# cloudtik/cloudtik

Hardware: AMD Instinct MI355X
Metric: bert_large_pretrain_tokens_per_sec (higher is better)
Workload: dtype bf16

## Files before the change

### cloudtik_amd/ops/csrc/bindings_lt.cpp

```cpp
#include <torch/extension.h>
#include <ATen/hip/HIPContext.h>
#include <ATen/hip/HIPContextLight.h>
#include <hipblaslt/hipblaslt.h>
#include <hipblaslt/hipblaslt-ext.hpp>
#include <map>
#include <vector>
#include <mutex>
#include <tuple>

namespace {

#define LT_CHECK(x)                                                                     \
  do {                                                                                  \
    hipblasStatus_t st_ = (x);                                                          \
    TORCH_CHECK(st_ == HIPBLAS_STATUS_SUCCESS, "hipBLASLt: ", #x, " failed: ", (int)st_); \
  } while (0)

using Key = std::tuple<long, long, long, long, long, long, long, long, long, int, int, int, int, int>;

struct Plan {
  hipblasLtMatmulDesc_t desc = nullptr;
  hipblasLtMatrixLayout_t a = nullptr, b = nullptr, c = nullptr, d = nullptr;
  hipblasLtMatmulAlgo_t algo;
  size_t ws = 0;
// ... 223 lines not shown
      tuned_ms = p.ok ? best : -1.0;
      it = g_bplans.emplace(key, p).first;
    }
    plan = &it->second;
  }
  if (!plan->ok) return -1.0;
  LT_CHECK(hipblasLtMatmul(handle, plan->desc, &al, B.data_ptr(), plan->a, A.data_ptr(), plan->b, &be, D.data_ptr(),
                           plan->d, D.data_ptr(), plan->d, &plan->algo, ws, plan->ws, stream));
  return tuned_ms;
}

extern "C" int ct_gemm_nt(const void*, long, const void*, long, void*, long, int, int, int, int, int, const void*,
                          void*, long, float*, int, hipStream_t, int);

static bool gemm_nt_impl(at::Tensor A, at::Tensor B, at::Tensor D, int64_t epi, bool accumulate,
                         c10::optional<at::Tensor> bias, c10::optional<at::Tensor> aux, c10::optional<at::Tensor> dbias,
                         bool b_kn) {
  TORCH_CHECK(A.is_cuda() && B.is_cuda() && D.is_cuda(), "gemm_nt: GPU tensors");
  TORCH_CHECK(A.scalar_type() == at::kBFloat16 && B.scalar_type() == at::kBFloat16 &&
              D.scalar_type() == at::kBFloat16, "gemm_nt: bf16 operands");
  TORCH_CHECK(rowmajor_ok(A) && rowmajor_ok(B) && rowmajor_ok(D), "gemm_nt: 2-D row-major operands");
  const long M = A.size(0), K = A.size(1), N = b_kn ? B.size(1) : B.size(0);
  TORCH_CHECK((b_kn ? B.size(0) : B.size(1)) == K && D.size(0) == M && D.size(1) == N, "gemm_nt: shape mismatch");
  const bool hb = bias.has_value() && bias->defined(), ha = aux.has_value() && aux->defined(),
             hd = dbias.has_value() && dbias->defined();
  if (hb) TORCH_CHECK(bias->scalar_type() == at::kBFloat16 && bias->is_contiguous() && bias->numel() == N,
                      "gemm_nt: bias");
  if (ha) TORCH_CHECK(aux->scalar_type() == at::kBFloat16 && rowmajor_ok(*aux) && aux->size(0) == M &&
                      aux->size(1) == N, "gemm_nt: aux");
  const long drows = hd && N > 0 ? dbias->numel() / N : 1;
  if (hd) TORCH_CHECK(dbias->scalar_type() == at::kFloat && dbias->is_contiguous() && dbias->numel() == drows * N &&
                      drows >= 1 && (drows & (drows - 1)) == 0, "gemm_nt: dbias must be [N] or [2^k, N] fp32");
  TORCH_CHECK((epi != 1 && epi != 6) || (hb && ha), "gemm_nt: epilogues 1 / 6 need bias and aux");
  TORCH_CHECK((epi != 2 && epi != 7) || ha, "gemm_nt: epilogues 2 / 7 need aux");
  int rc = ct_gemm_nt(A.data_ptr(), A.stride(0), B.data_ptr(), B.stride(0), D.data_ptr(), D.stride(0), (int)M,
                      (int)N, (int)K, (int)epi, accumulate ? 1 : 0, hb ? bias->data_ptr() : nullptr,
                      ha ? aux->data_ptr() : nullptr, ha ? aux->stride(0) : 0,
                      hd ? dbias->data_ptr<float>() : nullptr, b_kn ? 1 : 0, at::hip::getCurrentHIPStream().stream(),
                      (int)drows);
  return rc == 0;
}

bool gemm_nt(at::Tensor A, at::Tensor B, at::Tensor D, int64_t epi, bool accumulate, c10::optional<at::Tensor> bias,
             c10::optional<at::Tensor> aux, c10::optional<at::Tensor> dbias) {
  return gemm_nt_impl(A, B, D, epi, accumulate, bias, aux, dbias, false);
}

bool gemm_nn(at::Tensor A, at::Tensor B, at::Tensor D, int64_t epi, bool accumulate, c10::optional<at::Tensor> bias,
             c10::optional<at::Tensor> aux, c10::optional<at::Tensor> dbias) {
  return gemm_nt_impl(A, B, D, epi, accumulate, bias, aux, dbias, true);
}

extern "C" int ct_gemm_nt_stream(const void*, long, const void*, long, void*, long, int, int, int, int, const void*,
                                 int, int, int, hipStream_t);

bool gemm_nt_stream(at::Tensor A, at::Tensor B, at::Tensor D, c10::optional<at::Tensor> bias, bool b_kn,
                    int64_t wgs, bool accumulate) {
  TORCH_CHECK(A.is_cuda() && B.is_cuda() && D.is_cuda(), "gemm_nt_stream: GPU tensors");
  TORCH_CHECK(A.scalar_type() == at::kBFloat16 && B.scalar_type() == at::kBFloat16 &&
              D.scalar_type() == at::kBFloat16, "gemm_nt_stream: bf16 operands");
  TORCH_CHECK(rowmajor_ok(A) && rowmajor_ok(B) && rowmajor_ok(D), "gemm_nt_stream: 2-D row-major operands");
  const long M = A.size(0), K = A.size(1), N = b_kn ? B.size(1) : B.size(0);
  TORCH_CHECK((b_kn ? B.size(0) : B.size(1)) == K && D.size(0) == M && D.size(1) == N,
              "gemm_nt_stream: shape mismatch");
  const bool hb = bias.has_value() && bias->defined();
  if (hb) TORCH_CHECK(bias->scalar_type() == at::kBFloat16 && bias->is_contiguous() && bias->numel() == N,
                      "gemm_nt_stream: bias");
  int rc = ct_gemm_nt_stream(A.data_ptr(), A.stride(0), B.data_ptr(), B.stride(0), D.data_ptr(), D.stride(0),
                             (int)M, (int)N, (int)K, hb ? 5 : 0, hb ? bias->data_ptr() : nullptr, b_kn ? 1 : 0,
                             (int)wgs, accumulate ? 1 : 0, at::hip::getCurrentHIPStream().stream());
  return rc == 0;
}

extern "C" int ct_gemm_pp(const void*, long, const void*, long, void*, long, int, int, int, int, const void*, void*,
                          long, int, int, hipStream_t);

bool gemm_pp(at::Tensor A, at::Tensor B, at::Tensor D, int64_t epi, c10::optional<at::Tensor> bias,
             c10::optional<at::Tensor> aux, int64_t wgs, int64_t eslots) {
  TORCH_CHECK(A.is_cuda() && B.is_cuda() && D.is_cuda(), "gemm_pp: GPU tensors");
  TORCH_CHECK(A.scalar_type() == at::kBFloat16 && B.scalar_type() == at::kBFloat16 &&
              D.scalar_type() == at::kBFloat16, "gemm_pp: bf16 operands");
  TORCH_CHECK(rowmajor_ok(A) && rowmajor_ok(B) && rowmajor_ok(D), "gemm_pp: 2-D row-major operands");
  const long M = A.size(0), K = A.size(1), N = B.size(0);
  TORCH_CHECK(B.size(1) == K && D.size(0) == M && D.size(1) == N, "gemm_pp: shape mismatch");
  const bool hb = bias.has_value() && bias->defined();
  const bool ha = aux.has_value() && aux->defined();
  if (hb) TORCH_CHECK(bias->scalar_type() == at::kBFloat16 && bias->is_contiguous() && bias->numel() == N,
                      "gemm_pp: bias");
  if (ha) TORCH_CHECK(aux->scalar_type() == at::kBFloat16 && rowmajor_ok(*aux) && aux->size(0) == M &&
                      aux->size(1) == N, "gemm_pp: aux");
  int rc = ct_gemm_pp(A.data_ptr(), A.stride(0), B.data_ptr(), B.stride(0), D.data_ptr(), D.stride(0), (int)M, (int)N,
                      (int)K, (int)epi, hb ? bias->data_ptr() : nullptr, ha ? aux->data_ptr() : nullptr,
                      ha ? aux->stride(0) : 0, (int)wgs, (int)eslots, at::hip::getCurrentHIPStream().stream());
  return rc == 0;
}

extern "C" int ct_gemm_w4(const void*, long, const void*, long, void*, long, int, int, int, int, int, const void*, void*,
                          long, hipStream_t);

bool gemm_w4(at::Tensor A, at::Tensor B, at::Tensor D, int64_t epi, c10::optional<at::Tensor> bias,
             c10::optional<at::Tensor> aux) {
  TORCH_CHECK(A.is_cuda() && B.is_cuda() && D.is_cuda(), "gemm_w4: GPU tensors");
  TORCH_CHECK(A.scalar_type() == at::kBFloat16 && B.scalar_type() == at::kBFloat16 &&
              D.scalar_type() == at::kBFloat16, "gemm_w4: bf16 operands");
  TORCH_CHECK(rowmajor_ok(A) && rowmajor_ok(B) && rowmajor_ok(D), "gemm_w4: 2-D row-major operands");
  const long M = A.size(0), K = A.size(1), N = B.size(0);
  TORCH_CHECK(B.size(1) == K && D.size(0) == M && D.size(1) == N, "gemm_w4: shape mismatch");
  const bool hb = bias.has_value() && bias->defined();
  const bool ha = aux.has_value() && aux->defined();
  if (hb) TORCH_CHECK(bias->scalar_type() == at::kBFloat16 && bias->is_contiguous() && bias->numel() == N,
                      "gemm_w4: bias");
  if (ha) TORCH_CHECK(aux->scalar_type() == at::kBFloat16 && rowmajor_ok(*aux) && aux->size(0) == M &&
                      aux->size(1) == N, "gemm_w4: aux");
  int rc = ct_gemm_w4(A.data_ptr(), A.stride(0), B.data_ptr(), B.stride(0), D.data_ptr(), D.stride(0), (int)M, (int)N,
                      (int)K, (int)epi, 0, hb ? bias->data_ptr() : nullptr, ha ? aux->data_ptr() : nullptr,
                      ha ? aux->stride(0) : 0, at::hip::getCurrentHIPStream().stream());
  return rc == 0;
}

extern "C" int ct_gemm_tn2(const void*, long, const void*, long, void*, long, int, int, long, int, int, float*,
                           hipStream_t);

static void check_tn_problem(const char* who, const at::Tensor& A, const at::Tensor& B, const at::Tensor& out,
// ... 23 lines not shown
                     (int)splits, accumulate ? 1 : 0, biasg, at::hip::getCurrentHIPStream().stream()) == 0;
}

bool gemm_tn2(at::Tensor A, at::Tensor B, at::Tensor out, int64_t splits, bool accumulate) {
  return gemm_tn2_impl(A, B, out, splits, accumulate, nullptr);
}

bool gemm_tn2_bias(at::Tensor A, at::Tensor B, at::Tensor out, int64_t splits, bool accumulate, at::Tensor biasg) {
  TORCH_CHECK(biasg.is_cuda() && biasg.scalar_type() == at::kFloat && biasg.is_contiguous() &&
              biasg.numel() == splits * A.size(1), "gemm_tn2_bias: fp32 [splits, M] bias partials");
  return gemm_tn2_impl(A, B, out, splits, accumulate, biasg.data_ptr<float>());
}

extern "C" int ct_gemm_tn_group(int, const void* const*, const long*, const void* const*, const long*, float* const*,
                                float* const*, const int*, const int*, long, int, hipStream_t);

bool gemm_tn_group(std::vector<at::Tensor> A, std::vector<at::Tensor> B, std::vector<at::Tensor> P,
                   std::vector<c10::optional<at::Tensor>> biasg, int64_t splits) {
  const size_t n = A.size();
  TORCH_CHECK(n >= 1 && B.size() == n && P.size() == n && biasg.size() == n, "gemm_tn_group: list lengths");
  std::vector<const void*> a(n), b(n);
  std::vector<float*> p(n), bg(n);
  std::vector<long> lda(n), ldb(n);
  std::vector<int> Ms(n), Ns(n);
  const long K = A[0].dim() == 2 ? A[0].size(0) : -1;
  for (size_t i = 0; i < n; ++i) {
    check_tn_problem("gemm_tn_group", A[i], B[i], P[i], K, splits, true);
    const long M = A[i].size(1), N = B[i].size(1);
    const bool hb = biasg[i].has_value() && biasg[i]->defined();
    if (hb)
      TORCH_CHECK(biasg[i]->is_cuda() && biasg[i]->scalar_type() == at::kFloat && biasg[i]->is_contiguous() &&
                  biasg[i]->numel() == splits * M, "gemm_tn_group: fp32 [splits, M] bias partials");
    a[i] = A[i].data_ptr();
    b[i] = B[i].data_ptr();
    p[i] = P[i].data_ptr<float>();
    bg[i] = hb ? biasg[i]->data_ptr<float>() : nullptr;
    lda[i] = A[i].stride(0);
    ldb[i] = B[i].stride(0);
    Ms[i] = (int)M;
    Ns[i] = (int)N;
  }
  return ct_gemm_tn_group((int)n, a.data(), lda.data(), b.data(), ldb.data(), p.data(), bg.data(), Ms.data(),
                          Ns.data(), K, (int)std::min<int64_t>(splits, 1 << 30),
                          at::hip::getCurrentHIPStream().stream()) == 0;
}

void register_lt(pybind11::module& m) {
  m.def("gemm_tn_group", &gemm_tn_group, "several gemm_tn2 problems sharing K and the slice count, one launch");
  m.def("gemm_tn2", &gemm_tn2, "weight-gradient GEMM A^T @ B (token-major operands) on the MFMA kernel");
  m.def("gemm_tn2_bias", &gemm_tn2_bias, "gemm_tn2 + per-split column sums of A (bias gradient)");
  m.def("gemm_nt", &gemm_nt, "hand-written MFMA GEMM A @ B^T with fused epilogues");
  m.def("gemm_nt_stream", &gemm_nt_stream, "streamed persistent MFMA GEMM A @ B^T / A @ B (+ bias)",
        pybind11::arg("A"), pybind11::arg("B"), pybind11::arg("D"), pybind11::arg("bias") = pybind11::none(), pybind11::arg("b_kn") = false,
        pybind11::arg("wgs") = 0, pybind11::arg("accumulate") = false);
  m.def("gemm_pp", &gemm_pp, "paired-tile persistent MFMA GEMM A @ B^T (epilogue of one tile beside another's K loop)",
        pybind11::arg("A"), pybind11::arg("B"), pybind11::arg("D"), pybind11::arg("epi") = 0,
        pybind11::arg("bias") = pybind11::none(), pybind11::arg("aux") = pybind11::none(), pybind11::arg("wgs") = 0,
        pybind11::arg("eslots") = 4);
  m.def("gemm_w4", &gemm_w4, "four-wave MFMA GEMM A @ B^T (128 x 128 per wave, AGPR-resident accumulators)",
        pybind11::arg("A"), pybind11::arg("B"), pybind11::arg("D"), pybind11::arg("epi") = 0,
        pybind11::arg("bias") = pybind11::none(), pybind11::arg("aux") = pybind11::none());
  m.def("gemm_nn", &gemm_nn, "hand-written MFMA GEMM A @ B (B stored [K, N]) with fused epilogues");
  m.def("lt_matmul", &lt_matmul, "hipBLASLt matmul with epilogue (row-major semantics)");
  m.def("lt_bmm_tuned", &lt_bmm_tuned, "strided-batched hipBLASLt GEMM, algorithm picked by timing all solutions");
}
```

### cloudtik_amd/ops/csrc/gemm_nt.hip

```cpp
#include "common.h"
#include <algorithm>
#include <cstdlib>

namespace ct {

typedef __attribute__((ext_vector_type(8))) short nt_s16x8;
typedef __attribute__((address_space(3))) nt_s16x8 nt_lds_s16x8;
typedef __attribute__((address_space(3))) void nt_lds_void;

constexpr int NT_BM = 256, NT_BN = 256, NT_BK = 64, NT_THREADS = 512;
constexpr int NT_ROWB = NT_BK * 2;
constexpr int NT_HALF = 128 * NT_ROWB;
constexpr int NT_BUF = 4 * NT_HALF;

enum { NT_EPI_PLAIN = 0, NT_EPI_BIAS_GELU_AUX = 1, NT_EPI_DGELU_BGRAD = 2, NT_EPI_F32_SLAB = 3, NT_EPI_NONE = 4,
       NT_EPI_BIAS = 5, NT_EPI_BIAS_GELU_DAUX = 6, NT_EPI_MUL_AUX_BGRAD = 7 };

struct NtArgs {
  const bf16_t* A;
  const bf16_t* B;
  bf16_t* D;
  const bf16_t* bias;
  bf16_t* aux;
  float* dbias;
// ... 124 lines not shown
    const long krow = c.kbase + k0 + piece * 4;
    const bf16_t* base;
    unsigned off;
    if (slot == 0 || slot == 3) {
      if constexpr (!Ly::AT) {
        base = c.A + (c.m0 + ((piece >> 3) << 7) + (slot == 3 ? 64 : 0) + (piece & 7) * 8) * c.lda + k0;
        off = i ? c.offa1 : c.offa0;
      } else {
        base = c.A + krow * c.lda + c.m0 + (slot == 3 ? 64 : 0);
        off = c.offa0;
      }
    } else {
      if constexpr (!Ly::BT) {
        base = c.B + (c.n0 + ((piece >> 2) << 6) + (slot == 2 ? 32 : 0) + (piece & 3) * 8) * c.ldb + k0;
        off = i ? c.offb1 : c.offb0;
      } else {
        base = c.B + krow * c.ldb + c.n0 + (slot == 2 ? 32 : 0);
        off = c.offb0;
      }
    }
    nt_glds16s(base, off, dst + piece * 1024);
  }
}

template <int N>
__device__ __forceinline__ void nt_vm() {
  asm volatile("s_waitcnt vmcnt(%0)" ::"n"(N) : "memory");
}

template <int I0, int J0>
__device__ __forceinline__ void nt_quad(f32x4 (&acc)[8][4], const nt_s16x8 (&fa)[4][2], const nt_s16x8 (&fb)[2][2]) {
#pragma unroll
  for (int ks = 0; ks < 2; ++ks)
#pragma unroll
    for (int i = 0; i < 4; ++i)
#pragma unroll
      for (int j = 0; j < 2; ++j)
        acc[I0 + i][J0 + j] = __builtin_amdgcn_mfma_f32_16x16x32_bf16((bf16x8_t)fb[j][ks], (bf16x8_t)fa[i][ks],
                                                                       acc[I0 + i][J0 + j], 0, 0, 0);
}

template <int LAY>
__device__ __forceinline__ void nt_stage_v(const NtCtx& c, int v) {
  const int T = (v + 6) >> 2, slot = (v + 6) & 3;
  nt_stage_slot<LAY>(c, (long)T * NT_BK, slot, c.lds + (T & 1) * NT_BUF + slot * NT_HALF);
}

template <bool KMAJOR>
__device__ __forceinline__ nt_s16x8 nt_fragment(const char* img, int r0, int ks, int lane) {
  if constexpr (KMAJOR) return tn_frag(img, r0, ks, lane);
  else return nt_frag(img, r0, ks, lane);
}

template <int POS>
struct NtPlan {
  static constexpr bool issue(int q) { return POS == 0 || (POS == 1 && q < 2); }
  static constexpr int wait(int q) {
    return POS == 0 ? 8 : (POS == 1 ? (q < 2 ? 8 : (q == 2 ? 6 : 4)) : (q == 0 ? 2 : 0));
  }
};

template <int POS, int DIAG, int LAY, bool BIASG>
__device__ __forceinline__ void nt_ktile(const NtCtx& c, int t, f32x4 (&acc)[8][4], nt_s16x8 (&fa)[2][4][2],
                                         nt_s16x8 (&fb)[2][2][2], f32x4 (&accb)[2]) {
  const char* buf = c.lds + (t & 1) * NT_BUF;
  constexpr bool WAIT = DIAG == 0, BAR = DIAG != 2;
  constexpr bool DMA = DIAG == 0 || DIAG == 3;
  using P = NtPlan<POS>;
#define NT_PHASE_TAIL(Q, I0, J0, FA, FB)                                             \
  if constexpr (DMA && P::issue(Q)) nt_stage_v<LAY>(c, 4 * t + Q);                   \
  if constexpr (WAIT) nt_vm<P::wait(Q)>();                                           \
  if constexpr (BAR) nt_mma_begin(); else asm volatile("s_waitcnt lgkmcnt(0)" ::: "memory"); \
  if (c.half != (J0 == 0 ? 2 : 1)) nt_quad<I0, J0>(acc, FA, FB);                     \
  if constexpr (BIASG && (Q == 0 || Q == 2)) nt_quad_bias<Q, I0>(accb, FA, c.biasw); \
  if constexpr (BAR) nt_mma_end(); else __builtin_amdgcn_sched_barrier(0);
#pragma unroll
  for (int j = 0; j < 2; ++j)
#pragma unroll
    for (int ks = 0; ks < 2; ++ks) fb[0][j][ks] = nt_fragment<NtLay<LAY>::BT>(buf + 1 * NT_HALF, c.rb + j * 16, ks, c.lane);
#pragma unroll
  for (int i = 0; i < 4; ++i)
#pragma unroll
    for (int ks = 0; ks < 2; ++ks) fa[0][i][ks] = nt_fragment<NtLay<LAY>::AT>(buf + 0 * NT_HALF, c.ra + i * 16, ks, c.lane);
  NT_PHASE_TAIL(0, 0, 0, fa[0], fb[0])
#pragma unroll
  for (int j = 0; j < 2; ++j)
#pragma unroll
    for (int ks = 0; ks < 2; ++ks) fb[1][j][ks] = nt_fragment<NtLay<LAY>::BT>(buf + 2 * NT_HALF, c.rb + j * 16, ks, c.lane);
  NT_PHASE_TAIL(1, 0, 2, fa[0], fb[1])
#pragma unroll
  for (int i = 0; i < 4; ++i)
#pragma unroll
    for (int ks = 0; ks < 2; ++ks) fa[1][i][ks] = nt_fragment<NtLay<LAY>::AT>(buf + 3 * NT_HALF, c.ra + i * 16, ks, c.lane);
  NT_PHASE_TAIL(2, 4, 2, fa[1], fb[1])
  NT_PHASE_TAIL(3, 4, 0, fa[1], fb[0])
#undef NT_PHASE_TAIL
}

__device__ __forceinline__ u16x8 nt_pair_swap(u16x4 x, u16x4 y) {
  const uint2 xv = __builtin_bit_cast(uint2, x), yv = __builtin_bit_cast(uint2, y);
  const auto s0 = __builtin_amdgcn_permlane16_swap(xv.x, yv.x, false, false);
  const auto s1 = __builtin_amdgcn_permlane16_swap(xv.y, yv.y, false, false);
  const uint4 v = {s0[0], s1[0], s0[1], s1[1]};
  return __builtin_bit_cast(u16x8, v);
}

__device__ __forceinline__ void nt_pair_unswap(u16x8 v, u16x4& x, u16x4& y) {
  const uint4 w = __builtin_bit_cast(uint4, v);
  const auto r0 = __builtin_amdgcn_permlane16_swap(w.x, w.z, false, false);
  const auto r1 = __builtin_amdgcn_permlane16_swap(w.y, w.w, false, false);
  x = __builtin_bit_cast(u16x4, uint2{r0[0], r1[0]});
// ... 283 lines not shown
  if (!SPLIT && a.group_m > 1) {
    const int gsz = a.group_m * tiles_n;
    const int g = L / gsz, r = L - g * gsz;
    tm = g * a.group_m + r % a.group_m;
    tn = r / a.group_m;
  } else {
    tm = L / tiles_n;
    tn = L % tiles_n;
  }
  nt_tile<EPI, BGRAD, DIAG, LAY, BIASG>(a, lds, tm, tn, split, half, true);
}

constexpr int NT_GROUP_MAX = 4;

struct NtGroupArgs {
  const bf16_t* A[NT_GROUP_MAX];
  const bf16_t* B[NT_GROUP_MAX];
  float* P[NT_GROUP_MAX];
  float* biasg[NT_GROUP_MAX];
  long lda[NT_GROUP_MAX], ldb[NT_GROUP_MAX];
  int M[NT_GROUP_MAX], N[NT_GROUP_MAX];
  int tile_base[NT_GROUP_MAX];
  int tiles_total;
  int K, tsplit;
};

template <int EPI, bool BGRAD, int DIAG, int LAY, bool BIASG>
__global__ void __launch_bounds__(NT_THREADS, 1) gemm_nt_kernel(NtGroupArgs g) {
  static_assert(EPI == NT_EPI_F32_SLAB && !BGRAD && DIAG == 0 && LAY == 1 && BIASG,
                "the grouped form exists for TN split-K slabs with runtime bias sums only");
  __shared__ __attribute__((aligned(1024))) char lds[2 * NT_BUF];
  int L = xcd_remap(blockIdx.x, gridDim.x);
  const int split = L / g.tiles_total;
  L -= split * g.tiles_total;
  NtArgs a{};
  a.A = g.A[0]; a.B = g.B[0]; a.P = g.P[0]; a.biasg = g.biasg[0];
  a.lda = g.lda[0]; a.ldb = g.ldb[0]; a.M = g.M[0]; a.N = g.N[0];
  int base = 0;
#pragma unroll
  for (int i = 1; i < NT_GROUP_MAX; ++i)
    if (L >= g.tile_base[i]) {
      a.A = g.A[i]; a.B = g.B[i]; a.P = g.P[i]; a.biasg = g.biasg[i];
      a.lda = g.lda[i]; a.ldb = g.ldb[i]; a.M = g.M[i]; a.N = g.N[i];
      base = g.tile_base[i];
    }
  L -= base;
  a.K = g.K;
  a.tsplit = g.tsplit;
  const int tiles_n = a.N / NT_BN;
  const int tm = L / tiles_n, tn = L % tiles_n;
  nt_tile<EPI, BGRAD, DIAG, LAY, BIASG>(a, lds, tm, tn, split, 0, a.biasg != nullptr);
}

struct NtStream {
  int nk;
  int total_k;
  int tiles_n, tiles, P, wg, my_tiles;
  __device__ __forceinline__ void tile_origin(int j, long& m0, long& n0) const {
    const int L = xcd_remap(j * P + wg, tiles);
    m0 = (long)(L / tiles_n) * NT_BM;
    n0 = (long)(L % tiles_n) * NT_BN;
  }
};

struct NtKCur {
  int j, k;
  long ka, kb;
  const bf16_t* arow;
  const bf16_t* brow;
};

struct NtSOff {
  long pa[2], pb[2];
  long a64, b32;
};

template <int LAY>
__device__ __forceinline__ void nt_kcur_set(const NtCtx& c, const NtStream& st, NtKCur& q, int j) {
  q.j = j;
  q.k = 0;
  q.ka = 0;
  q.kb = 0;
  if (j < st.my_tiles) {
    long m0, n0;
    st.tile_origin(j, m0, n0);
    q.arow = c.A + m0 * c.lda;
    q.brow = NtLay<LAY>::BT ? c.B + n0 : c.B + n0 * c.ldb;
  }
}

template <int LAY>
__device__ __forceinline__ void nt_kcur_next(const NtCtx& c, const NtStream& st, NtKCur& q) {
  if (++q.k == st.nk) {
    nt_kcur_set<LAY>(c, st, q, q.j + 1);
  } else {
    q.ka += NT_BK;
    q.kb += NtLay<LAY>::BT ? NT_BK * c.ldb : NT_BK;
  }
}

template <int LAY, int SLOT>
__device__ __forceinline__ void nt_stage_kt(const NtCtx& c, const NtSOff& so, const NtKCur& q, char* buf) {
  using Ly = NtLay<LAY>;
  static_assert(!Ly::AT, "streamed kernel: NT / NN layouts only");
  char* dst = buf + SLOT * NT_HALF;
#pragma unroll
  for (int i = 0; i < 2; ++i) {
    const int piece = c.wave * 2 + i;
    const bf16_t* base;
    unsigned off;
    if constexpr (SLOT == 0 || SLOT == 3) {
      base = q.arow + so.pa[i] + (SLOT == 3 ? so.a64 : 0) + q.ka;
      off = i ? c.offa1 : c.offa0;
    } else {
      base = q.brow + so.pb[i] + (SLOT == 2 ? so.b32 : 0) + q.kb;
      off = Ly::BT ? c.offb0 : (i ? c.offb1 : c.offb0);
    }
    nt_glds16s(base, off, dst + piece * 1024);
  }
}

template <int POS, int LAY>
__device__ __forceinline__ void nt_ktile_stream(const NtCtx& c, const NtSOff& so, const NtKCur& q1,
                                                const NtKCur& q2, int t, f32x4 (&acc)[8][4],
                                                nt_s16x8 (&fa)[2][4][2], nt_s16x8 (&fb)[2][2][2]) {
  const char* buf = c.lds + (t & 1) * NT_BUF;
  char* nbuf = c.lds + ((t + 1) & 1) * NT_BUF;
  char* cbuf = c.lds + (t & 1) * NT_BUF;
  using P = NtPlan<POS>;
#define NT_SPHASE_TAIL(Q, I0, J0, FA, FB)                                                  \
  if constexpr (P::issue(Q)) {                                                             \
    if constexpr (Q == 0) nt_stage_kt<LAY, 2>(c, so, q1, nbuf);                            \
    else if constexpr (Q == 1) nt_stage_kt<LAY, 3>(c, so, q1, nbuf);                       \
    else if constexpr (Q == 2) nt_stage_kt<LAY, 0>(c, so, q2, cbuf);                       \
    else nt_stage_kt<LAY, 1>(c, so, q2, cbuf);                                             \
  }                                                                                        \
  nt_vm<P::wait(Q)>();                                                                     \
  nt_mma_begin();                                                                          \
  nt_quad<I0, J0>(acc, FA, FB);                                                            \
  nt_mma_end();
#pragma unroll
  for (int j = 0; j < 2; ++j)
#pragma unroll
    for (int ks = 0; ks < 2; ++ks) fb[0][j][ks] = nt_fragment<NtLay<LAY>::BT>(buf + 1 * NT_HALF, c.rb + j * 16, ks, c.lane);
#pragma unroll
  for (int i = 0; i < 4; ++i)
#pragma unroll
    for (int ks = 0; ks < 2; ++ks) fa[0][i][ks] = nt_fragment<false>(buf + 0 * NT_HALF, c.ra + i * 16, ks, c.lane);
  NT_SPHASE_TAIL(0, 0, 0, fa[0], fb[0])
#pragma unroll
  for (int j = 0; j < 2; ++j)
#pragma unroll
    for (int ks = 0; ks < 2; ++ks) fb[1][j][ks] = nt_fragment<NtLay<LAY>::BT>(buf + 2 * NT_HALF, c.rb + j * 16, ks, c.lane);
  NT_SPHASE_TAIL(1, 0, 2, fa[0], fb[1])
#pragma unroll
  for (int i = 0; i < 4; ++i)
#pragma unroll
    for (int ks = 0; ks < 2; ++ks) fa[1][i][ks] = nt_fragment<false>(buf + 3 * NT_HALF, c.ra + i * 16, ks, c.lane);
  NT_SPHASE_TAIL(2, 4, 2, fa[1], fb[1])
  NT_SPHASE_TAIL(3, 4, 0, fa[1], fb[0])
#undef NT_SPHASE_TAIL
}

template <int EPI, int LAY>
__global__ void __launch_bounds__(NT_THREADS, 1) gemm_nt_stream_kernel(NtArgs a, int P) {
  __shared__ __attribute__((aligned(1024))) char lds[2 * NT_BUF];
  const int tiles_n = a.N / NT_BN;
  const int tiles = (a.M / NT_BM) * tiles_n;
  const int wg = blockIdx.x;
  const int my_tiles = wg < tiles ? (tiles - wg + P - 1) / P : 0;
  const int nk = a.K / NT_BK;
  NtStream st{nk, my_tiles * nk, tiles_n, tiles, P, wg, my_tiles};
  if (my_tiles == 0) return;
  const int tid = threadIdx.x, lane = tid & 63;
  const int wave = __builtin_amdgcn_readfirstlane(tid >> 6);
  const int wr = wave >> 2, wc = wave & 3;
  NtCtx c{a.A, a.B, a.lda, a.ldb, 0, 0, 0, lds, wave, lane, wr * 64, wc * 32, 0, 0, 0, 0, -1, 0};
  c.offa0 = nt_lane_off(a.lda, 0, lane);
  c.offa1 = nt_lane_off(a.lda, 1, lane);
  if constexpr (NtLay<LAY>::BT) {
    c.offb0 = c.offb1 = tn_lane_off(a.ldb, wave, lane, false);
  } else {
    c.offb0 = nt_lane_off(a.ldb, 0, lane);
    c.offb1 = nt_lane_off(a.ldb, 1, lane);
  }
  NtSOff so;
#pragma unroll
  for (int i = 0; i < 2; ++i) {
    const int piece = wave * 2 + i;
    so.pa[i] = (long)(((piece >> 3) << 7) + (piece & 7) * 8) * a.lda;
    so.pb[i] = NtLay<LAY>::BT ? (long)piece * 4 * a.ldb : (long)(((piece >> 2) << 6) + (piece & 3) * 8) * a.ldb;
  }
  so.a64 = 64 * a.lda;
  so.b32 = NtLay<LAY>::BT ? 32 : 32 * a.ldb;

  f32x4 acc[8][4];
#pragma unroll
  for (int i = 0; i < 8; ++i)
#pragma unroll
    for (int j = 0; j < 4; ++j) acc[i][j] = f32x4{0.f, 0.f, 0.f, 0.f};
  long m0, n0;
  st.tile_origin(0, m0, n0);
  NtEpiPre<4> epre;
  nt_preload_bias<EPI, 4>(a, n0 + wc * 64 + (lane >> 4) * 4, epre);
  nt_s16x8 fa[2][4][2];
  nt_s16x8 fb[2][2][2];

  NtKCur q1, q2;
  nt_kcur_set<LAY>(c, st, q1, 0);
  nt_stage_kt<LAY, 0>(c, so, q1, lds);
  nt_stage_kt<LAY, 1>(c, so, q1, lds);
  nt_stage_kt<LAY, 2>(c, so, q1, lds);
  nt_stage_kt<LAY, 3>(c, so, q1, lds);
  nt_kcur_next<LAY>(c, st, q1);
  if (st.total_k > 1) {
    nt_stage_kt<LAY, 0>(c, so, q1, lds + NT_BUF);
    nt_stage_kt<LAY, 1>(c, so, q1, lds + NT_BUF);
    nt_vm<8>();
  } else {
    nt_vm<4>();
  }
  q2 = q1;
  nt_kcur_next<LAY>(c, st, q2);
  nt_bar();
  if (wr == 1) nt_bar();

  int jt = 0, kin = 0;
  auto finish_k = [&]() {
    q1 = q2;
    nt_kcur_next<LAY>(c, st, q2);
    if (++kin != nk) return;
    const long emrow = m0 + wr * 128 + (lane & 15), encol = n0 + wc * 64 + (lane >> 4) * 4;
    nt_epilogue<EPI, false, 4>(a, acc, emrow, encol, lane, 0, epre);
#pragma unroll
    for (int i = 0; i < 8; ++i)
#pragma unroll
      for (int j = 0; j < 4; ++j) acc[i][j] = f32x4{0.f, 0.f, 0.f, 0.f};
    kin = 0;
    if (++jt < my_tiles) {
      st.tile_origin(jt, m0, n0);
      nt_preload_bias<EPI, 4>(a, n0 + wc * 64 + (lane >> 4) * 4, epre);
    }
  };
  const int T = st.total_k;
  int t = 0;
  for (; t < T - 2; ++t) {
    nt_ktile_stream<0, LAY>(c, so, q1, q2, t, acc, fa, fb);
    finish_k();
  }
  if (T >= 2) {
    nt_ktile_stream<1, LAY>(c, so, q1, q2, t, acc, fa, fb);
    finish_k();
    ++t;
  }
  nt_ktile_stream<2, LAY>(c, so, q1, q2, t, acc, fa, fb);
  finish_k();
  if (wr == 0) nt_bar();
}


__device__ __forceinline__ void w4_glds16s(const void* sbase, unsigned voff, const char* lds_wave_base) {
  const unsigned la = __builtin_amdgcn_readfirstlane((unsigned)(uintptr_t)(nt_lds_void*)lds_wave_base);
  const uint64_t sb = (uint64_t)(uint32_t)__builtin_amdgcn_readfirstlane((unsigned)(uintptr_t)sbase) |
                      ((uint64_t)(uint32_t)__builtin_amdgcn_readfirstlane((unsigned)((uintptr_t)sbase >> 32)) << 32);
  asm volatile("s_mov_b32 m0, %2\n\ts_nop 4\n\tglobal_load_lds_dwordx4 %0, %1" ::"v"(voff), "s"(sb), "s"(la)
               : "memory", "m0");
}


template <bool FIRST>
__device__ __forceinline__ void w4_mfma(f32x4& c, const nt_s16x8& b, const nt_s16x8& a) {
  if constexpr (FIRST)
    asm volatile("v_mfma_f32_16x16x32_bf16 %0, %1, %2, 0" : "=a"(c) : "v"(b), "v"(a));
  else
    asm volatile("v_mfma_f32_16x16x32_bf16 %0, %1, %2, %0" : "+a"(c) : "v"(b), "v"(a));
}

struct W4Frags {
  nt_s16x8 a[8], b[8];
};

template <int DIAG, bool RD, bool DMA, bool FIRST = false>
__device__ __forceinline__ void w4_kstep(f32x4 (&acc)[8][8], const W4Frags& cur, W4Frags& nxt, const char* rimg,
                                         int ks, int wm, int wn, int lane, char* dimg,
                                         const bf16_t* abase, const bf16_t* bbase, long lda, long ldb, long k0,
                                         unsigned oa0, unsigned oa1, unsigned ob0, unsigned ob1, int wave) {
#pragma unroll
  for (int q = 0; q < 64; ++q) {
    const int i = q >> 3, j = q & 7;
    w4_mfma<FIRST>(acc[i][j], cur.b[j], cur.a[i]);
    if constexpr (DIAG != 1 && DMA) {
      if (q < 16) {
        const int pc = q & 7;
        if (q < 8) w4_glds16s(abase + 8 * pc * lda + k0, (pc & 1) ? oa1 : oa0, dimg + (8 * wave + pc) * 1024);
        else w4_glds16s(bbase + 8 * pc * ldb + k0, (pc & 1) ? ob1 : ob0, dimg + 32768 + (8 * wave + pc) * 1024);
      }
    }
    if (RD && q >= 16 && (q - 16) % 3 == 0 && (q - 16) / 3 < 16) {
      const int f = (q - 16) / 3;
      const int lo = ((ks * 4 + (lane >> 4)) ^ (((lane & 15) >> 1) & 7)) << 4;
      if (f < 8) nxt.a[f] = *(const nt_lds_s16x8*)(rimg + (wm * 128 + (lane & 15)) * NT_ROWB + lo + f * 16 * NT_ROWB);
      else nxt.b[f - 8] = *(const nt_lds_s16x8*)(rimg + 32768 + (wn * 128 + (lane & 15)) * NT_ROWB + lo +
                                                 (f - 8) * 16 * NT_ROWB);
    }
    __builtin_amdgcn_sched_barrier(0);
  }
}

template <int EPI, bool BGRAD, int DIAG = 0>
// ... 44 lines not shown
  nt_bar();
#pragma unroll
  for (int f = 0; f < 8; ++f) {
    s0.a[f] = nt_frag(lds, wm * 128 + 16 * f, 0, lane);
    s0.b[f] = nt_frag(lds + 32768, wn * 128 + 16 * f, 0, lane);
  }
#define W4_TILE(FIRST0, RD1, DMA1, WAITV)                                                          \
  do {                                                                                               \
    const char* img = lds + (t & 1) * NT_BUF;                                                        \
    w4_kstep<DIAG, true, false, FIRST0>(acc, s0, s1, img, 1, wm, wn, lane, nullptr, abase, bbase,    \
                                        a.lda, a.ldb, 0, oa0, oa1, ob0, ob1, wave);                  \
    asm volatile("s_waitcnt lgkmcnt(0)" ::: "memory");                                               \
    if constexpr (DIAG == 0 && WAITV) nt_vm<0>();                                                    \
    nt_bar();                                                                                        \
    w4_kstep<DIAG, RD1, DMA1>(acc, s1, s0, lds + ((t + 1) & 1) * NT_BUF, 0, wm, wn, lane,            \
                              lds + (t & 1) * NT_BUF, abase, bbase, a.lda, a.ldb, (long)(t + 2) * NT_BK, \
                              oa0, oa1, ob0, ob1, wave);                                             \
  } while (0)
  int t = 0;
  if (nk == 1) {
    W4_TILE(true, false, false, false);
  } else {
    if (nk == 2) W4_TILE(true, true, false, true);
    else W4_TILE(true, true, true, true);
    for (t = 1; t < nk - 2; ++t) W4_TILE(false, true, true, true);
    if (nk >= 3) {
      W4_TILE(false, true, false, true);
      ++t;
    }
    W4_TILE(false, false, false, false);
  }
#undef W4_TILE
  __builtin_amdgcn_sched_barrier(0);
  asm volatile("s_nop 7\n\ts_nop 7\n\ts_nop 7" ::: "memory");
  __builtin_amdgcn_sched_barrier(0);
  nt_epilogue<EPI, BGRAD, 8, false>(a, acc, emrow, encol, lane, 0, epre);
}

}

using namespace ct;

static int nt_cu_count() {
  static int n = [] {
    int dev = 0, v = 0;
    if (hipGetDevice(&dev) != hipSuccess ||
        hipDeviceGetAttribute(&v, hipDeviceAttributeMultiprocessorCount, dev) != hipSuccess || v <= 0) v = 256;
    return v;
  }();
  return n;
}

extern "C" int ct_gemm_nt_stream(const void* A, long lda, const void* B, long ldb, void* D, long ldd, int M, int N,
                                 int K, int epi, const void* bias, int b_kn, int wgs, int accumulate,
                                 hipStream_t stream) {
  if (M <= 0 || N <= 0 || K <= 0 || M % NT_BM || N % NT_BN || K % NT_BK) return 1;
  if (lda % 8 || ldb % 8 || ldd % 8 || lda < K || ldb < (b_kn ? N : K) || ldd < N) return 2;
  if (((uintptr_t)A & 15) || ((uintptr_t)B & 15) || ((uintptr_t)D & 15)) return 3;
  if (epi != 0 && epi != 5) return 6;
  if (epi == 5 && (!bias || ((uintptr_t)bias & 7))) return 4;
  const long tiles = (long)(M / NT_BM) * (N / NT_BN);
  if (tiles > (1L << 30)) return 5;
  const int P = (int)std::min<long>(tiles, wgs > 0 ? wgs : nt_cu_count());
  if (accumulate && epi != 0) return 6;
  NtArgs a{(const bf16_t*)A, (const bf16_t*)B, (bf16_t*)D, (const bf16_t*)bias, nullptr, nullptr, nullptr,
           nullptr, lda, ldb, ldd, 0, 0, M, N, K, accumulate ? 1 : 0};
  if (epi == 5) {
    if (b_kn) gemm_nt_stream_kernel<NT_EPI_BIAS, 2><<<P, NT_THREADS, 0, stream>>>(a, P);
    else gemm_nt_stream_kernel<NT_EPI_BIAS, 0><<<P, NT_THREADS, 0, stream>>>(a, P);
  } else {
    if (b_kn) gemm_nt_stream_kernel<NT_EPI_PLAIN, 2><<<P, NT_THREADS, 0, stream>>>(a, P);
    else gemm_nt_stream_kernel<NT_EPI_PLAIN, 0><<<P, NT_THREADS, 0, stream>>>(a, P);
  }
  return hipGetLastError() == hipSuccess ? 0 : 7;
}

extern "C" int ct_gemm_nt(const void* A, long lda, const void* B, long ldb, void* D, long ldd, int M, int N, int K,
                          int epi, int accumulate, const void* bias, void* aux, long ldaux, float* dbias, int b_kn,
                          hipStream_t stream, int dbias_rows) {
  if (dbias_rows < 1 || (dbias_rows & (dbias_rows - 1))) return 6;
  if (M <= 0 || N <= 0 || K <= 0 || M % NT_BM || N % NT_BN || K % NT_BK) return 1;
  if (lda % 8 || ldb % 8 || ldd % 8 || lda < K || ldb < (b_kn ? N : K) || ldd < N) return 2;
  if (((uintptr_t)A & 15) || ((uintptr_t)B & 15) || ((uintptr_t)D & 15)) return 3;
  if ((epi == 1 || epi == 6) && (!bias || !aux || ((uintptr_t)bias & 7))) return 4;
  if (epi == 5 && (!bias || ((uintptr_t)bias & 7))) return 4;
  if ((epi == 1 || epi == 2 || epi == 6 || epi == 7) && (!aux || ((uintptr_t)aux & 15) || ldaux % 8 || ldaux < N))
    return 4;
  if (bias && ((uintptr_t)bias & 7)) return 4;
  const long tiles = (long)(M / NT_BM) * (N / NT_BN);
  if (tiles > (1L << 30)) return 5;
  static const int stag_env = [] { const char* e = getenv("CLOUDTIK_AMD_GEMM_STAGGER"); return e ? atoi(e) : 0; }();
  int H = 0;
  if (stag_env > 0) H = (int)std::min<long>(stag_env, tiles / 2);
  else if (stag_env < 0 && tiles >= 2L * nt_cu_count()) H = nt_cu_count() / 2;
  const long blocks = tiles + H;
  static const int gm_env = [] { const char* e = getenv("CLOUDTIK_AMD_GEMM_GROUP_M"); return e ? atoi(e) : 4; }();
  const int gm = (gm_env > 1 && (M / NT_BM) % gm_env == 0) ? gm_env : 1;
  NtArgs a{(const bf16_t*)A, (const bf16_t*)B, (bf16_t*)D, (const bf16_t*)bias, (bf16_t*)aux, dbias, nullptr,
           nullptr, lda, ldb, ldd, ldaux, 0, M, N, K, accumulate, H, gm, dbias_rows};
  static const int diag = [] { const char* e = getenv("CLOUDTIK_AMD_GEMM_DIAG"); return e ? atoi(e) : 0; }();
  if (diag == 4) {
    if (b_kn) gemm_nt_kernel<NT_EPI_NONE, false, 0, 2><<<(int)blocks, NT_THREADS, 0, stream>>>(a);
    else gemm_nt_kernel<NT_EPI_NONE, false, 0, 0><<<(int)blocks, NT_THREADS, 0, stream>>>(a);
    return 0;
  }
  if (diag && !b_kn) {
    if (diag == 1) gemm_nt_kernel<0, false, 1><<<(int)blocks, NT_THREADS, 0, stream>>>(a);
    else if (diag == 2) gemm_nt_kernel<0, false, 2><<<(int)blocks, NT_THREADS, 0, stream>>>(a);
    else gemm_nt_kernel<0, false, 3><<<(int)blocks, NT_THREADS, 0, stream>>>(a);
    return 0;
  }
#define NT_LAUNCH(E, BG)                                                                  \
  do {                                                                                    \
    if (b_kn) gemm_nt_kernel<E, BG, 0, 2><<<(int)blocks, NT_THREADS, 0, stream>>>(a);     \
    else gemm_nt_kernel<E, BG, 0, 0><<<(int)blocks, NT_THREADS, 0, stream>>>(a);          \
  } while (0)
  switch (epi) {
    case 0: NT_LAUNCH(0, false); break;
    case 1: NT_LAUNCH(1, false); break;
    case 2:
// ... 107 lines not shown
```

### cloudtik_amd/ops/transformer.py

```python
from __future__ import annotations

import math
import os

import torch

from cloudtik_amd.ops.linear import grad_ready as _ready
from cloudtik_amd.ops.linear import issue_wgrads, wgrad_group_enabled, wgrad_side


def _C():
    from cloudtik_amd import ops
    return ops.require_native()


_FUSED_FFN_DGRAD = os.environ.get("CLOUDTIK_AMD_FUSED_FFN_DGRAD", "1") == "1"


_FUSED_FFN_FWD = os.environ.get("CLOUDTIK_AMD_FUSED_FFN_FWD", "1") == "1"


_STORE_DGELU = os.environ.get("CLOUDTIK_AMD_FFN_STORE_DGELU", "1") == "1"


def _fused_ffn1(C, x2, W1, b1f):
    T, H = x2.shape
    F = W1.shape[0]
    if T % 256 or F % 256 or H % 64 or b1f.dtype != torch.bfloat16:
        return None
    aux = torch.empty(T, F, device=x2.device, dtype=x2.dtype)
    h = torch.empty_like(aux)
    epi = 6 if _STORE_DGELU else 1
    if not C.gemm_nt(x2, W1, h, epi, False, b1f, aux, None):
        return None
    return aux, h, ("dgelu" if epi == 6 else "z")


_DB_ACC = {}


_DB_ROWS = int(os.environ.get("CLOUDTIK_AMD_DBIAS_ROWS", "1"))


def _zeroed_acc(device, F, rows=1):
    key = (device, F, rows)
    t = _DB_ACC.get(key)
    if t is None:
        t = _DB_ACC[key] = torch.zeros(rows, F, device=device, dtype=torch.float32)
    return t


_FFN_BGRAD_IN_WGRAD = os.environ.get("CLOUDTIK_AMD_FFN_BGRAD_IN_WGRAD", "1") == "1"
_LN_FROM_Y = os.environ.get("CLOUDTIK_AMD_LN_FROM_Y", "1") == "1"


def _fused_ffn_dgrad(C, df, W2, z, b1f, db1f, dgelu=False):
    T, F = z.shape
    if T % 256 or F % 256 or df.shape[1] % 64:
        return None
    dz = torch.empty_like(z)
    if db1f is None:
        return dz if C.gemm_nn(df, W2, dz, 7 if dgelu else 2, False, None if dgelu else b1f, z, None) else None
    direct = db1f.dtype == torch.bfloat16 and db1f.is_contiguous()
    rows = _DB_ROWS if direct else 1
    db = _zeroed_acc(z.device, F, rows) if direct else torch.zeros(1, F, device=z.device, dtype=torch.float32)
    if not C.gemm_nn(df, W2, dz, 7 if dgelu else 2, False, None if dgelu else b1f, z, db):
        return None
    if direct:
        C.splitk_reduce_clear(db, db1f, True)
    else:
        db1f.add_(db[0])
    return dz


_STREAM_SITES = os.environ.get("CLOUDTIK_AMD_STREAM_GEMM", "")
_STREAM_SITES = ({"qkv", "wo", "ffn2", "do", "dx_attn", "dx_ffn"} if _STREAM_SITES == "all"
                 else {t for t in _STREAM_SITES.split(",") if t})


_ONETILE_ENV = os.environ.get("CLOUDTIK_AMD_ONETILE_GEMM")
_ONETILE_SITES = ({"qkv", "wo", "ffn2", "do", "dx_attn", "dx_ffn"} if _ONETILE_ENV == "all"
                  else {t for t in (_ONETILE_ENV or "").split(",") if t})
_ONETILE_INLINE_SITES = {"do", "dx_attn", "dx_ffn"} if _ONETILE_ENV is None else set()


def _onetile(site, side: bool) -> bool:
    if site in _ONETILE_SITES:
        return True
    return site in _ONETILE_INLINE_SITES and not side


def _stream_mm(site, A, B, b_kn, bias=None, out=None, side=True):
    stream = site in _STREAM_SITES
    if not stream and not _onetile(site, side):
        return None
    M, K = A.shape
    N = B.shape[1] if b_kn else B.shape[0]
    if M % 256 or N % 256 or K % 64 or not A.is_contiguous() or not B.is_contiguous():
        return None
    if bias is not None and (bias.dtype != torch.bfloat16 or not bias.is_contiguous()):
        return None
    acc = out is not None
    D = out if acc else torch.empty(M, N, device=A.device, dtype=A.dtype)
    C = _C()
    if stream:
        ok = C.gemm_nt_stream(A, B, D, bias, b_kn, 0, acc)
    elif b_kn:
        ok = bias is None and C.gemm_nn(A, B, D, 0, acc, None, None, None)
    else:
        ok = C.gemm_nt(A, B, D, 5 if bias is not None else 0, acc, bias, None, None)
    return D if ok else None


def _flat(p) -> bool:
# ... 188 lines not shown
```

Before: 469,500.

## Route FFN GELU GEMMs through streamed persistent kernel with overlapped epilogue

```diff
diff --git a/cloudtik_amd/ops/csrc/bindings_lt.cpp b/cloudtik_amd/ops/csrc/bindings_lt.cpp
--- a/cloudtik_amd/ops/csrc/bindings_lt.cpp
+++ b/cloudtik_amd/ops/csrc/bindings_lt.cpp
@@ -299,10 +299,10 @@
 }
 
 extern "C" int ct_gemm_nt_stream(const void*, long, const void*, long, void*, long, int, int, int, int, const void*,
-                                 int, int, int, hipStream_t);
+                                 int, int, int, void*, long, hipStream_t);
 
 bool gemm_nt_stream(at::Tensor A, at::Tensor B, at::Tensor D, c10::optional<at::Tensor> bias, bool b_kn,
-                    int64_t wgs, bool accumulate) {
+                    int64_t wgs, bool accumulate, int64_t epi, c10::optional<at::Tensor> aux) {
   TORCH_CHECK(A.is_cuda() && B.is_cuda() && D.is_cuda(), "gemm_nt_stream: GPU tensors");
   TORCH_CHECK(A.scalar_type() == at::kBFloat16 && B.scalar_type() == at::kBFloat16 &&
               D.scalar_type() == at::kBFloat16, "gemm_nt_stream: bf16 operands");
@@ -310,12 +310,16 @@
   const long M = A.size(0), K = A.size(1), N = b_kn ? B.size(1) : B.size(0);
   TORCH_CHECK((b_kn ? B.size(0) : B.size(1)) == K && D.size(0) == M && D.size(1) == N,
               "gemm_nt_stream: shape mismatch");
-  const bool hb = bias.has_value() && bias->defined();
+  const bool hb = bias.has_value() && bias->defined(), ha = aux.has_value() && aux->defined();
   if (hb) TORCH_CHECK(bias->scalar_type() == at::kBFloat16 && bias->is_contiguous() && bias->numel() == N,
                       "gemm_nt_stream: bias");
+  if (ha) TORCH_CHECK(aux->is_cuda() && aux->scalar_type() == at::kBFloat16 && rowmajor_ok(*aux) &&
+                      aux->size(0) == M && aux->size(1) == N, "gemm_nt_stream: aux");
+  if (epi < 0) epi = hb ? 5 : 0;
   int rc = ct_gemm_nt_stream(A.data_ptr(), A.stride(0), B.data_ptr(), B.stride(0), D.data_ptr(), D.stride(0),
-                             (int)M, (int)N, (int)K, hb ? 5 : 0, hb ? bias->data_ptr() : nullptr, b_kn ? 1 : 0,
-                             (int)wgs, accumulate ? 1 : 0, at::hip::getCurrentHIPStream().stream());
+                             (int)M, (int)N, (int)K, (int)epi, hb ? bias->data_ptr() : nullptr, b_kn ? 1 : 0,
+                             (int)wgs, accumulate ? 1 : 0, ha ? aux->data_ptr() : nullptr,
+                             ha ? aux->stride(0) : 0, at::hip::getCurrentHIPStream().stream());
   return rc == 0;
 }
 
@@ -445,7 +449,8 @@
   m.def("gemm_nt", &gemm_nt, "hand-written MFMA GEMM A @ B^T with fused epilogues");
   m.def("gemm_nt_stream", &gemm_nt_stream, "streamed persistent MFMA GEMM A @ B^T / A @ B (+ bias)",
         pybind11::arg("A"), pybind11::arg("B"), pybind11::arg("D"), pybind11::arg("bias") = pybind11::none(), pybind11::arg("b_kn") = false,
-        pybind11::arg("wgs") = 0, pybind11::arg("accumulate") = false);
+        pybind11::arg("wgs") = 0, pybind11::arg("accumulate") = false, pybind11::arg("epi") = -1,
+        pybind11::arg("aux") = pybind11::none());
   m.def("gemm_pp", &gemm_pp, "paired-tile persistent MFMA GEMM A @ B^T (epilogue of one tile beside another's K loop)",
         pybind11::arg("A"), pybind11::arg("B"), pybind11::arg("D"), pybind11::arg("epi") = 0,
         pybind11::arg("bias") = pybind11::none(), pybind11::arg("aux") = pybind11::none(), pybind11::arg("wgs") = 0,
diff --git a/cloudtik_amd/ops/csrc/gemm_nt.hip b/cloudtik_amd/ops/csrc/gemm_nt.hip
--- a/cloudtik_amd/ops/csrc/gemm_nt.hip
+++ b/cloudtik_amd/ops/csrc/gemm_nt.hip
@@ -200,11 +200,13 @@
   else return nt_frag(img, r0, ks, lane);
 }
 
-template <int POS>
+template <int POS, int E = 0>
 struct NtPlan {
-  static constexpr bool issue(int q) { return POS == 0 || (POS == 1 && q < 2); }
+  static_assert(POS == 3 ? (E >= 0 && 8 + E <= 63) : E == 0, "vmcnt is a 6-bit field");
+  static constexpr bool issue(int q) { return POS == 0 || POS == 3 || (POS == 1 && q < 2); }
   static constexpr int wait(int q) {
-    return POS == 0 ? 8 : (POS == 1 ? (q < 2 ? 8 : (q == 2 ? 6 : 4)) : (q == 0 ? 2 : 0));
+    return POS == 3 ? 8 + E
+                    : (POS == 0 ? 8 : (POS == 1 ? (q < 2 ? 8 : (q == 2 ? 6 : 4)) : (q == 0 ? 2 : 0)));
   }
 };
 
@@ -594,6 +596,14 @@
   nt_tile<EPI, BGRAD, DIAG, LAY, BIASG>(a, lds, tm, tn, split, 0, a.biasg != nullptr);
 }
 
+template <int EPI>
+struct NtStreamE {
+  static constexpr int stores = EPI == NT_EPI_BIAS_GELU_DAUX ? 32 : 16;
+  static constexpr int bias_loads = (EPI == NT_EPI_BIAS || EPI == NT_EPI_BIAS_GELU_DAUX) ? 4 : 0;
+  static constexpr int value = stores + bias_loads;
+  static_assert(EPI == NT_EPI_PLAIN || EPI == NT_EPI_BIAS || EPI == NT_EPI_BIAS_GELU_DAUX ||
+                EPI == NT_EPI_MUL_AUX_BGRAD, "streamed kernel: epilogues 0, 5, 6, 7");
+};
 struct NtStream {
   int nk;
   int total_k;
@@ -662,14 +672,14 @@
   }
 }
 
-template <int POS, int LAY>
+template <int POS, int LAY, int E = 0>
 __device__ __forceinline__ void nt_ktile_stream(const NtCtx& c, const NtSOff& so, const NtKCur& q1,
                                                 const NtKCur& q2, int t, f32x4 (&acc)[8][4],
                                                 nt_s16x8 (&fa)[2][4][2], nt_s16x8 (&fb)[2][2][2]) {
   const char* buf = c.lds + (t & 1) * NT_BUF;
   char* nbuf = c.lds + ((t + 1) & 1) * NT_BUF;
   char* cbuf = c.lds + (t & 1) * NT_BUF;
-  using P = NtPlan<POS>;
+  using P = NtPlan<POS, E>;
 #define NT_SPHASE_TAIL(Q, I0, J0, FA, FB)                                                  \
   if constexpr (P::issue(Q)) {                                                             \
     if constexpr (Q == 0) nt_stage_kt<LAY, 2>(c, so, q1, nbuf);                            \
@@ -758,45 +768,80 @@
   if (st.total_k > 1) {
     nt_stage_kt<LAY, 0>(c, so, q1, lds + NT_BUF);
     nt_stage_kt<LAY, 1>(c, so, q1, lds + NT_BUF);
-    nt_vm<8>();
-  } else {
-    nt_vm<4>();
+  }
+  nt_vm<0>();
+  if constexpr (NtStreamE<EPI>::bias_loads > 0) {
+#pragma unroll
+    for (int j = 0; j < 4; ++j) asm volatile("" : "+v"(epre.bias[j]));
   }
   q2 = q1;
   nt_kcur_next<LAY>(c, st, q2);
   nt_bar();
   if (wr == 1) nt_bar();
 
-  int jt = 0, kin = 0;
-  auto finish_k = [&]() {
+  int jt = 0, t = 0;
+  auto next_k = [&]() {
     q1 = q2;
     nt_kcur_next<LAY>(c, st, q2);
-    if (++kin != nk) return;
+    ++t;
+  };
+  auto finish_tile = [&]() {
     const long emrow = m0 + wr * 128 + (lane & 15), encol = n0 + wc * 64 + (lane >> 4) * 4;
-    nt_epilogue<EPI, false, 4>(a, acc, emrow, encol, lane, 0, epre);
-#pragma unroll
-    for (int i = 0; i < 8; ++i)
-#pragma unroll
-      for (int j = 0; j < 4; ++j) acc[i][j] = f32x4{0.f, 0.f, 0.f, 0.f};
-    kin = 0;
+    constexpr bool HAS_BIAS = NtStreamE<EPI>::bias_loads > 0;
+    NtEpiPre<4> nxt;
+    if constexpr (HAS_BIAS) {
+#pragma unroll
+      for (int j = 0; j < 4; ++j) nxt.bias[j] = epre.bias[j];
+    }
     if (++jt < my_tiles) {
       st.tile_origin(jt, m0, n0);
-      nt_preload_bias<EPI, 4>(a, n0 + wc * 64 + (lane >> 4) * 4, epre);
+      nt_preload_bias<EPI, 4>(a, n0 + wc * 64 + (lane >> 4) * 4, nxt);
+    }
+    nt_epilogue<EPI, false, 4>(a, acc, emrow, encol, lane, 0, epre);
+#pragma unroll
+    for (int i = 0; i < 8; ++i)
+#pragma unroll
+      for (int j = 0; j < 4; ++j) acc[i][j] = f32x4{0.f, 0.f, 0.f, 0.f};
+    if constexpr (HAS_BIAS) {
+#pragma unroll
+      for (int j = 0; j < 4; ++j) epre.bias[j] = nxt.bias[j];
     }
   };
+  constexpr int E = NtStreamE<EPI>::value;
   const int T = st.total_k;
-  int t = 0;
-  for (; t < T - 2; ++t) {
-    nt_ktile_stream<0, LAY>(c, so, q1, q2, t, acc, fa, fb);
-    finish_k();
+  const int body_tiles = my_tiles - (nk >= 2 || my_tiles < 2 ? 1 : 2);
+  if (nk >= 2) {
+    while (jt < body_tiles) {
+      nt_ktile_stream<3, LAY, E>(c, so, q1, q2, t, acc, fa, fb);
+      next_k();
+      for (int k = 1; k < nk; ++k) {
+        nt_ktile_stream<0, LAY>(c, so, q1, q2, t, acc, fa, fb);
+        next_k();
+      }
+      finish_tile();
+    }
+    if (nk >= 3) {
+      nt_ktile_stream<3, LAY, E>(c, so, q1, q2, t, acc, fa, fb);
+      next_k();
+      for (int k = 1; k < nk - 2; ++k) {
+        nt_ktile_stream<0, LAY>(c, so, q1, q2, t, acc, fa, fb);
+        next_k();
+      }
+    }
+  } else {
+    while (jt < body_tiles) {
+      nt_ktile_stream<0, LAY>(c, so, q1, q2, t, acc, fa, fb);
+      next_k();
+      finish_tile();
+    }
   }
   if (T >= 2) {
     nt_ktile_stream<1, LAY>(c, so, q1, q2, t, acc, fa, fb);
-    finish_k();
-    ++t;
+    next_k();
+    if (nk == 1) finish_tile();
   }
   nt_ktile_stream<2, LAY>(c, so, q1, q2, t, acc, fa, fb);
-  finish_k();
+  finish_tile();
   if (wr == 0) nt_bar();
 }
 
@@ -947,20 +992,26 @@
 }
 
 extern "C" int ct_gemm_nt_stream(const void* A, long lda, const void* B, long ldb, void* D, long ldd, int M, int N,
-                                 int K, int epi, const void* bias, int b_kn, int wgs, int accumulate,
-                                 hipStream_t stream) {
+                                 int K, int epi, const void* bias, int b_kn, int wgs, int accumulate, void* aux,
+                                 long ldaux, hipStream_t stream) {
   if (M <= 0 || N <= 0 || K <= 0 || M % NT_BM || N % NT_BN || K % NT_BK) return 1;
   if (lda % 8 || ldb % 8 || ldd % 8 || lda < K || ldb < (b_kn ? N : K) || ldd < N) return 2;
   if (((uintptr_t)A & 15) || ((uintptr_t)B & 15) || ((uintptr_t)D & 15)) return 3;
-  if (epi != 0 && epi != 5) return 6;
-  if (epi == 5 && (!bias || ((uintptr_t)bias & 7))) return 4;
+  if (epi != 0 && epi != 5 && epi != 6 && epi != 7) return 6;
+  if ((epi == 6 && b_kn) || (epi == 7 && !b_kn)) return 6;
+  if ((epi == 5 || epi == 6) && (!bias || ((uintptr_t)bias & 7))) return 4;
+  if ((epi == 6 || epi == 7) && (!aux || ((uintptr_t)aux & 15) || ldaux % 8 || ldaux < N)) return 4;
   const long tiles = (long)(M / NT_BM) * (N / NT_BN);
   if (tiles > (1L << 30)) return 5;
   const int P = (int)std::min<long>(tiles, wgs > 0 ? wgs : nt_cu_count());
   if (accumulate && epi != 0) return 6;
-  NtArgs a{(const bf16_t*)A, (const bf16_t*)B, (bf16_t*)D, (const bf16_t*)bias, nullptr, nullptr, nullptr,
-           nullptr, lda, ldb, ldd, 0, 0, M, N, K, accumulate ? 1 : 0};
-  if (epi == 5) {
+  NtArgs a{(const bf16_t*)A, (const bf16_t*)B, (bf16_t*)D, (const bf16_t*)bias, (bf16_t*)aux, nullptr, nullptr,
+           nullptr, lda, ldb, ldd, ldaux, 0, M, N, K, accumulate ? 1 : 0};
+  if (epi == 6) {
+    gemm_nt_stream_kernel<NT_EPI_BIAS_GELU_DAUX, 0><<<P, NT_THREADS, 0, stream>>>(a, P);
+  } else if (epi == 7) {
+    gemm_nt_stream_kernel<NT_EPI_MUL_AUX_BGRAD, 2><<<P, NT_THREADS, 0, stream>>>(a, P);
+  } else if (epi == 5) {
     if (b_kn) gemm_nt_stream_kernel<NT_EPI_BIAS, 2><<<P, NT_THREADS, 0, stream>>>(a, P);
     else gemm_nt_stream_kernel<NT_EPI_BIAS, 0><<<P, NT_THREADS, 0, stream>>>(a, P);
   } else {
diff --git a/cloudtik_amd/ops/transformer.py b/cloudtik_amd/ops/transformer.py
--- a/cloudtik_amd/ops/transformer.py
+++ b/cloudtik_amd/ops/transformer.py
@@ -21,6 +21,19 @@
 
 
 _STORE_DGELU = os.environ.get("CLOUDTIK_AMD_FFN_STORE_DGELU", "1") == "1"
+
+
+_STREAM_FFN = os.environ.get("CLOUDTIK_AMD_STREAM_FFN", "1")
+_STREAM_FFN_MIN_TILES = None
+
+
+def _stream_ffn(site, T, F, device) -> bool:
+    if _STREAM_FFN != "1" and _STREAM_FFN != site:
+        return False
+    floor = _STREAM_FFN_MIN_TILES
+    if floor is None:
+        floor = torch.cuda.get_device_properties(device).multi_processor_count
+    return (T // 256) * (F // 256) > floor
 
 
 def _fused_ffn1(C, x2, W1, b1f):
@@ -31,6 +44,9 @@
     aux = torch.empty(T, F, device=x2.device, dtype=x2.dtype)
     h = torch.empty_like(aux)
     epi = 6 if _STORE_DGELU else 1
+    if (epi == 6 and _stream_ffn("fwd", T, F, x2.device)
+            and C.gemm_nt_stream(x2, W1, h, b1f, False, 0, False, epi=6, aux=aux)):
+        return aux, h, "dgelu"
     if not C.gemm_nt(x2, W1, h, epi, False, b1f, aux, None):
         return None
     return aux, h, ("dgelu" if epi == 6 else "z")
@@ -60,6 +76,9 @@
         return None
     dz = torch.empty_like(z)
     if db1f is None:
+        if (dgelu and _stream_ffn("dgrad", T, F, z.device)
+                and C.gemm_nt_stream(df, W2, dz, None, True, 0, False, epi=7, aux=z)):
+            return dz
         return dz if C.gemm_nn(df, W2, dz, 7 if dgelu else 2, False, None if dgelu else b1f, z, None) else None
     direct = db1f.dtype == torch.bfloat16 and db1f.is_contiguous()
     rows = _DB_ROWS if direct else 1
```

Result: faster. 476,100 (median of 6 runs) (+1.4%).
